# CHAINNEVERLIU/Pytorch-RL-EnhancedStableBaselines

Hardware: AMD Instinct MI355X
Metric: env-steps/sec (SAC, two-series CSTR, 4096 vec-envs) at 1/2/4/8 GPUs (higher is better)
Workload: dtype f32; 1 GPU; SAC MlpPolicy class defaults on 4096 vectorised two-series CSTR envs per GPU (obs 4/act 2, euler, batch 256, ring 244x4096, 1 gradient step per vec-step; hipGraph replay, 8 iterations per graph); n_envs_per_gpu=4096, global_batch=256, parallelism=dp1, hip_graph=True, hip_graph_requested=True, graph_unroll=8, blas=rocblas, n_updates=2370

## Files before the change

include/cstr_rl_hip.h:

```cpp
#ifndef CSTR_RL_HIP_H
#define CSTR_RL_HIP_H

#include <stdint.h>

#ifdef __cplusplus
extern "C" {
#endif

#define CSTR_ABI_VERSION 5

#define CSTR_OK 0
#define CSTR_E_BADARG (-1)
#define CSTR_E_UNSUPPORTED (-2)

#define CSTR_INTEGRATOR_EULER 0
#define CSTR_INTEGRATOR_RK4 1

typedef void *cstr_stream_t;

typedef struct cstr_coef {
    float q_v1, q_v2, cf, tf, tcf, k0, neg_e, r_gas, hk, rho_cp, cool1, cool2, neg_ua1, neg_ua2, rho_c, c_pc, dt;
    float s_lo[4], s_hi[4], s_span[4];
    float a_lo[2], a_hi[2], a_span[2];
    float target_c2, conc_span;
// ... 327 lines not shown
                         const cstr_sac_head_fin_t *fin, int tiles, cstr_stream_t stream);

typedef struct cstr_chain_root {
    int32_t mode, batch;
    float gamma, scale;
    const float *q_part[4];
    const float *b3[4];
    int32_t n_parts, reserved;
    const float *next_logp, *rew, *done;
    const float *ent_coef;
    const float *logp;
    float *target_out;
    float *q_out;
    float *gq_out;
    float *loss_out, *loss_sum;
    cstr_alpha_part_t alpha;
    uint64_t *rng_ctl;
    uint64_t rng_advance;
    int64_t *adam_advance[2];
    double adam_beta1[2], adam_beta2[2];
} cstr_chain_root_t;
int cstr_q_chain_bwd_f32(const cstr_chain_net_t *nets, int n_nets, const cstr_chain_root_t *root, int w_in, int obs_dim, int h1, int h2,
                         float *dz2, float *dz1, float *gact_part, int tiles, cstr_stream_t stream);

int cstr_chain_sum_parts_f32(const float *part, int n_parts, int64_t rows, int cols, float *out, int64_t out_stride, cstr_stream_t stream);

int cstr_sac_actor_chain_bwd_f32(const cstr_sac_actor_t *actor, const float *gact_part, int n_nets, int n_parts, const float *ent_coef,
                                 const float *x_pi, const float *params, const float *eps, const float *a_h1, const float *a_h2,
                                 float *g_params, float *dz2, float *dz1, int64_t batch, int kind, int tiles, cstr_stream_t stream);

#define CSTR_BCQ_MAX_LATENT 256
#define CSTR_BCQ_MAX_ACT 64
#define CSTR_BCQ_MAX_SAMPLES 4096
#define CSTR_BCQ_MAX_ROWS 16777216
int cstr_bcq_latent_fwd_f32(const float *params, int64_t ldp, const float *obs, int64_t ldo, const float *eps_in, uint64_t *rng_ctl,
                            float *xdec, int64_t ldx, float *std_out, float *eps_out, int64_t batch, int obs_dim, int latent,
                            cstr_stream_t stream);
int cstr_bcq_vae_loss_f32(const float *recon, int64_t ldr, const float *act, int64_t lda, const float *params, int64_t ldp,
                          const float *std, int64_t batch, int act_dim, int latent, float *g_recon, float *g_mean, float *g_std,
                          float *loss_out, float *loss_sum, cstr_stream_t stream);
int cstr_bcq_latent_bwd_f32(const float *g_z, int64_t ldg, const float *g_mean_kl, const float *g_std_kl, const float *params, int64_t ldp,
                            const float *std, const float *eps, float *g_params, int64_t batch, int latent, cstr_stream_t stream);
int cstr_bcq_expand_f32(const float *state, int64_t lds, int64_t n_states, int samples, int obs_dim, int latent, const float *noise,
                        uint64_t *rng_ctl, float clip, float *xdec, int64_t ldx, float *xa, int64_t lda, float *xb, int64_t ldb,
                        cstr_stream_t stream);
int cstr_bcq_perturb_fwd_f32(const float *a_vae, int64_t lda, const float *p, int64_t ldp, float max_perturbation, float *out, int64_t ldo,
// ... 141 lines not shown
```

pytorch-rl-enhancedstablebaselines_amd/core/_native.py:

```python
import ctypes as C
import os
from typing import Optional

_PKG_ROOT = os.path.dirname(os.path.dirname(os.path.abspath(__file__)))
LIB_PATH = os.environ.get("CSTR_LIB_PATH", os.path.join(_PKG_ROOT, "libcstr_rl_hip.so"))

INTEGRATORS = {"euler": 0, "rk4": 1}
RING_CTL_WORDS, ADAM_CTL_WORDS, MT_STATE_WORDS, PCG_STATE_WORDS, MAX_SAMPLE_BATCH = 4, 4, 628, 4, 16384
MAX_NOISE_PERIOD = 8
VECNORM_STATE_WORDS = 20
RNG_CTL_WORDS, MAX_HEAD_ACT, MAX_LINEAR_SETS, MAX_ADAM_SEGS = 16, 4, 16, 4
MAX_ENS_CRITICS = 16
SDE_MAX_LATENT, SDE_MAX_MATS = 4096, 65537
BCQ_MAX_LATENT, BCQ_MAX_ACT, BCQ_MAX_SAMPLES, BCQ_MAX_ROWS = 256, 64, 4096, 1 << 24
ROLLOUT_CTL_WORDS, PPO_WS_WORDS, PPO_MAX_BLOCKS, PPO_MAX_ROWS = 4, 1024, 64, 1 << 30
DQN_MAX_LEVELS = 16
HER_STRATEGIES = {"future": 0, "final": 1, "episode": 2}
HER_MAX_BATCH, HER_MAX_ROWS, HER_MAX_ENVS, HER_GOAL_TAG = 1024, 8192, 1 << 24, 0x90A17A67

SYMBOLS = (
    "cstr_abi_version", "cstr_error_string", "cstr_default_coef", "cstr_vec_step_f32", "cstr_reset_draw_f32",
    "cstr_replay_add_f32", "cstr_collect_step_f32", "cstr_collect_step_rng_f32", "cstr_mt19937_seed", "cstr_mt19937_normal_f32", "cstr_mt19937_normal_f64", "cstr_replay_sample_mt19937_f32", "cstr_replay_sample_packed_mt19937_f32", "cstr_replay_gather_packed_f32", "cstr_rollout_step_f32", "cstr_linear_act_fwd_gather_f32",
    "cstr_adam_multi_f32", "cstr_gaussian_head_fwd_f32", "cstr_gaussian_head_gemm_fwd_f32", "cstr_gaussian_head_bwd_f32", "cstr_gaussian_head_bwd_input_f32", "cstr_linear_act_fwd_f32", "cstr_linear_act_fwd_sets_f32", "cstr_linear_bwd_input_f32", "cstr_linear_bwd_weight_f32", "cstr_linear_bwd_weight_sets_f32", "cstr_td_twin_q_loss_f32", "cstr_policy_rows_fwd_f32", "cstr_policy_swizzle_f32", "cstr_target_smooth_f32", "cstr_linear_smooth_fwd_f32", "cstr_hidden_head_fwd_f32", "cstr_hidden_head_bwd_f32", "cstr_hidden_head_bwd_root_f32", "cstr_vecnorm_init_f64", "cstr_vecnorm_step_f64", "cstr_vecnorm_apply_f32",
    "cstr_td_target_min_f32", "cstr_polyak_f32", "cstr_adam_f32", "cstr_bias_act_fwd_f32", "cstr_bias_act_bwd_f32", "cstr_bias_act_bwd_rows_f32",
    "cstr_squashed_gaussian_fwd_f32", "cstr_squashed_gaussian_bwd_f32", "cstr_sac_alpha_f32", "cstr_twin_q_loss_f32",
    "cstr_sac_actor_loss_f32", "cstr_neg_mean_loss_f32", "cstr_td_ens_q_loss_f32", "cstr_sac_actor_ens_loss_f32",
    "cstr_sac_actor_chain_fwd_f32", "cstr_q_chain_fwd_f32", "cstr_q_chain_bwd_f32", "cstr_sac_actor_chain_bwd_f32",
    "cstr_linear_bwd_weight_adam_sets_f32", "cstr_wgrad_adam_lean", "cstr_wgrad_adam_tile_body", "cstr_chain_sum_parts_f32",
    "cstr_sde_draw_f32", "cstr_sde_head_fwd_f32", "cstr_sde_head_bwd_f32", "cstr_sde_param_grad_f32",
    "cstr_bcq_latent_fwd_f32", "cstr_bcq_vae_loss_f32", "cstr_bcq_latent_bwd_f32", "cstr_bcq_expand_f32", "cstr_bcq_perturb_fwd_f32",
    "cstr_bcq_perturb_bwd_f32", "cstr_bcq_target_f32", "cstr_bcq_select_f32",
    "cstr_diag_gaussian_act_f32", "cstr_rollout_add_f32", "cstr_gae_f32", "cstr_ppo_gather_f32", "cstr_ppo_loss_f32", "cstr_grad_clip_f32",
    "cstr_a2c_loss_f32", "cstr_rmsprop_f32",
    "cstr_mt19937_rand_flag_f64", "cstr_dqn_act_f32", "cstr_dqn_loss_f32",
    "cstr_eval_episodes_f32",
    "cstr_categorical_act_f32", "cstr_categorical_loss_f32",
    "cstr_goal_vec_step_f32", "cstr_her_add_f32", "cstr_her_sample_f32",
)


class Coef(C.Structure):
    _fields_ = [(n, C.c_float) for n in (
        "q_v1", "q_v2", "cf", "tf", "tcf", "k0", "neg_e", "r_gas", "hk", "rho_cp", "cool1", "cool2", "neg_ua1",
        "neg_ua2", "rho_c", "c_pc", "dt")] + [
        ("s_lo", C.c_float * 4), ("s_hi", C.c_float * 4), ("s_span", C.c_float * 4),
        ("a_lo", C.c_float * 2), ("a_hi", C.c_float * 2), ("a_span", C.c_float * 2),
        ("target_c2", C.c_float), ("conc_span", C.c_float), ("max_steps", C.c_int32)]


class Ring(C.Structure):
    _fields_ = [(n, C.c_void_p) for n in ("obs", "next_obs", "act", "rew", "done", "timeout")] + [
# ... 165 lines not shown
```

pytorch-rl-enhancedstablebaselines_amd/core/common/hip_ops.py:

```python
import ctypes as C
from typing import Optional

import torch as th

from core import _native as nv
from core._native import INTEGRATORS, check, ptr, stream_ptr


def _chk(t: th.Tensor, name: str, shape, dtype) -> th.Tensor:
    if not isinstance(t, th.Tensor):
        raise TypeError(f"{name}: expected a torch.Tensor, got {type(t)}")
    if not t.is_cuda:
        raise ValueError(f"{name}: must live in HBM (device tensor); got device {t.device}. No CPU fallback exists.")
    if t.device.index != th.cuda.current_device():
        raise ValueError(f"{name}: lives on {t.device}, the current device is cuda:{th.cuda.current_device()}")
    if t.dtype != dtype:
        raise ValueError(f"{name}: dtype {t.dtype}, expected {dtype}")
    if tuple(t.shape) != tuple(shape):
        raise ValueError(f"{name}: shape {tuple(t.shape)}, expected {tuple(shape)}")
    if not t.is_contiguous():
        raise ValueError(f"{name}: must be contiguous")
    return t


# ... 1231 lines not shown
               rng_advance=None, adam_advance=()) -> "nv.ChainRoot":
    part = nv.AlphaPart()
    if alpha is not None:
        part = nv.AlphaPart(alpha["log_alpha"].data_ptr(), alpha["logp_pi"].data_ptr(), float(alpha["target_entropy"]), alpha["grad_out"].data_ptr(),
                            alpha["ent_coef_out"].data_ptr(), *(_dp(alpha.get(k)) for k in ("loss_out", "loss_sum", "ent_coef_sum")))
    qp, bb = (C.c_void_p * 4)(), (C.c_void_p * 4)()
    for i, (q, b) in enumerate(zip(q_parts, b3s)):
        qp[i], bb[i] = q.data_ptr(), b.data_ptr()
    rc_ptr, adv = (None, 0) if rng_advance is None else (rng_advance[0].data_ptr(), int(rng_advance[1]))
    actl, ab1, ab2 = (C.c_void_p * 2)(), (C.c_double * 2)(), (C.c_double * 2)()
    for i, opt in enumerate(adam_advance):
        actl[i], (ab1[i], ab2[i]) = opt.ctl.data_ptr(), opt.param_groups[0]["betas"]
    return nv.ChainRoot({"td": 1, "sac_actor": 2, "neg_mean": 3}[mode], batch, float(gamma), float(scale), qp, bb, n_parts, 0, _dp(next_logp), _dp(rew),
                        _dp(done), None if alpha is not None else _dp(ent_coef), _dp(logp), _dp(target_out), _dp(q_out), _dp(gq_out), _dp(loss_out),
                        _dp(loss_sum), part, rc_ptr, adv, actl, ab1, ab2)


def q_chain_bwd(nets, root: "nv.ChainRoot", w_in: int, obs_dim: int, h1: int, h2: int, tiles: int, dz2=None, dz1=None, gact_part=None):
    arr = (nv.ChainNet * len(nets))(*nets)
    check(nv.lib().cstr_q_chain_bwd_f32(arr, C.c_int(len(nets)), C.byref(root), C.c_int(w_in), C.c_int(obs_dim), C.c_int(h1), C.c_int(h2), ptr(dz2),
                                        ptr(dz1), ptr(gact_part), C.c_int(tiles), stream_ptr()), "cstr_q_chain_bwd_f32")


def sac_actor_chain_bwd(actor: "nv.SacActorNet", gact_part, n_nets: int, n_parts: int, ent_coef, x_pi, params, eps, a_h1, a_h2, g_params, dz2, dz1,
                        batch: int, tiles: int, kind: int = 0):
    hn = actor.act_dim if kind == nv.CHAIN_HEAD_DETERMINISTIC else 2 * actor.act_dim
    _chk(gact_part, "gact_part", (n_nets, n_parts, batch, actor.act_dim), th.float32)
    _chk(g_params, "g_params", (batch, hn), th.float32), _chk(dz2, "dz2", (batch, actor.h2), th.float32)
    _chk(dz1, "dz1", (batch, actor.h1), th.float32)
    check(nv.lib().cstr_sac_actor_chain_bwd_f32(C.byref(actor), ptr(gact_part), C.c_int(n_nets), C.c_int(n_parts), ptr(ent_coef), ptr(x_pi), ptr(params),
                                                ptr(eps), ptr(a_h1), ptr(a_h2), ptr(g_params), ptr(dz2), ptr(dz1), C.c_int64(batch), C.c_int(kind),
                                                C.c_int(tiles), stream_ptr()), "cstr_sac_actor_chain_bwd_f32")


def chain_sum_parts(part, out):
    rows, cols = out.shape
    n_parts = part.numel() // (rows * cols)
    if part.numel() != n_parts * rows * cols or _f32c(part, "part") is None:
        raise ValueError("part: needs [n_parts, rows, cols]")
    if not (out.is_cuda and out.dtype == th.float32 and out.stride(1) == 1):
        raise ValueError("out: needs a float32 device matrix with unit inner stride")
    check(nv.lib().cstr_chain_sum_parts_f32(ptr(part), C.c_int(n_parts), C.c_int64(rows), C.c_int(cols), ptr(out), C.c_int64(out.stride(0)), stream_ptr()),
          "cstr_chain_sum_parts_f32")


PPO_SCALARS = ("policy_gradient_loss", "value_loss", "entropy_loss", "loss", "approx_kl", "clip_fraction")
# ... 313 lines not shown
```

pytorch-rl-enhancedstablebaselines_amd/csrc/cstr_chain.hip:

```cpp
#include <hip/hip_runtime.h>
#include <stdint.h>

#include "../../include/cstr_rl_hip.h"
#include "cstr_device.h"
#include "cstr_rng_device.h"

namespace {

using f32x4 = __attribute__((ext_vector_type(4))) float;
typedef unsigned int u32x4 __attribute__((ext_vector_type(4)));
constexpr int BUF_OOB = 0x40000000;
constexpr int CH_THREADS = 256, CH_WAVES = 4;
constexpr float LOG_STD_MIN = -20.0f, LOG_STD_MAX = 2.0f;
constexpr int MAX_A = CSTR_MAX_HEAD_ACT;

constexpr int SM_PART = 0;
constexpr int SM_RED = SM_PART + 3 * 64 * 4;
constexpr int SM_XS = SM_RED + 4 * 16 * 8;
constexpr int SM_GS = SM_XS + 16 * 16;
constexpr int SM_PANEL = SM_GS + 16 * 8;
static size_t chain_lds_bytes(int k, int w1_pad) { return (size_t)(SM_PANEL + 16 * (k + 4) + w1_pad * k) * sizeof(float); }

__device__ __forceinline__ __amdgpu_buffer_rsrc_t rsrc_of(const float *base, const int64_t floats)
{
// ... 778 lines not shown
#pragma unroll
        for (int e = 0; e < 4; ++e) a.dz1[((int64_t)g * B + m0 + 4 * h + e) * H1 + k0 + r] = d[e];
    }
    if (a.dz2) {
        const int cpg = (H2 + gridDim.x - 1) / gridDim.x;
#pragma unroll
        for (int i = 0; i < 2; ++i) {
            const int c = t + CH_THREADS * i;
            if (c < H2 && c / cpg == (int)blockIdx.x) {
#pragma unroll
                for (int row = 0; row < 16; ++row) a.dz2[((int64_t)g * B + m0 + row) * H2 + c] = y[i][row];
            }
        }
    }
    if (t < 16 && blockIdx.x == 0) {
        const int row = m0 + t;
        if (rt.q_out) rt.q_out[(int64_t)g * B + row] = o_q;
        if (rt.gq_out) rt.gq_out[(int64_t)g * B + row] = o_gq;
        if (rt.mode == 1 && g == 0 && rt.target_out) rt.target_out[row] = o_tq;
    }
    CH_STAMP(2, 7);
}

struct ActorBwdArgs {
    cstr_sac_actor_t net;
    const float *gact_part; int n_nets, n_parts; const float *ent_coef;
    const float *x_pi, *params, *eps, *a_h1, *a_h2;
    float *g_params, *dz2, *dz1;
    int batch, tiles, kind;
};

template <int D, int A, int NQ, int WX>
__global__ __launch_bounds__(CH_THREADS) void sac_actor_chain_bwd_kernel(const ActorBwdArgs a)
{
    extern __shared__ __align__(16) float smem[];
    constexpr int W = D + A;
    const int t = threadIdx.x, lane = t & 63, wave = t >> 6, r = lane & 15, h = lane >> 4;
    const int T = WX ? exact_tiles<NQ, WX>() : a.tiles, S = CH_WAVES / T, tile = wave % T, ks = wave / T;
    const int H1 = WX ? exact_h1<WX>() : a.net.h1, H2 = WX ? exact_h2<WX>() : a.net.h2, B = a.batch;
    const int k0 = (blockIdx.x * T + tile) * 16, m0 = blockIdx.y * 16;
    const bool col_ok = k0 + r < H1, det = a.kind == CSTR_CHAIN_HEAD_DETERMINISTIC;
    const int col = min(k0 + r, H1 - 1), HN = det ? A : 2 * A;
    float *gs = smem + SM_GS, *panel = smem + SM_PANEL;
    const int ld = H2 + 4;
    CH_STAMP(3, 0);
    float4 bq[NQ];
// ... 121 lines not shown
#define NQ_TOP_sac_actor_chain_bwd_kernel 16
#define CHAIN_DISPATCH(KERNEL, LAY, WXV, NQV, GRID, LDS, STREAM, ARGS)                             \
    do {                                                                                           \
        if ((LAY) == 0 && (WXV) == 1) CHAIN_NQ(KERNEL, 4, 2, 1, NQV, GRID, LDS, STREAM, ARGS);     \
        else if ((LAY) == 0 && (WXV) == 2) CHAIN_NQ(KERNEL, 4, 2, 2, NQV, GRID, LDS, STREAM, ARGS); \
        else if ((LAY) == 0) CHAIN_NQ(KERNEL, 4, 2, 0, NQV, GRID, LDS, STREAM, ARGS);              \
        else if ((LAY) == 1 && (WXV) == 1) CHAIN_NQ(KERNEL, 8, 2, 1, NQV, GRID, LDS, STREAM, ARGS); \
        else if ((LAY) == 1) CHAIN_NQ(KERNEL, 8, 2, 0, NQV, GRID, LDS, STREAM, ARGS);              \
        else if ((WXV) == 2) CHAIN_NQ(KERNEL, 8, 4, 2, NQV, GRID, LDS, STREAM, ARGS);              \
        else CHAIN_NQ(KERNEL, 8, 4, 0, NQV, GRID, LDS, STREAM, ARGS);                              \
    } while (0)

static int chain_wx(int h1, int h2, int tiles, int nq)
{
    static const bool off = getenv("CSTR_EXACT_SHAPES") && atoi(getenv("CSTR_EXACT_SHAPES")) == 0;
    if (off || (nq != 4 && nq != 8 && nq != 16)) return 0;
    if (h1 == 256 && h2 == 256 && nq == 4 * tiles) return 1;
    if (h1 == 400 && h2 == 300 && nq == 8 * tiles) return 2;
    return 0;
}

constexpr size_t CHAIN_LDS_LIMIT = 64 * 1024;

}

#ifdef CSTR_CHAIN_STAMPS
extern "C" int cstr_diag_chain_stamps(unsigned long long *host_out, int64_t words)
{
    return (int)hipMemcpyFromSymbol(host_out, HIP_SYMBOL(chain_stamps), (size_t)words * 8);
}
#endif

static int check_actor(const cstr_sac_actor_t *n)
{
    if (!n || !n->w1 || !n->b1 || !n->w2 || !n->b2 || !n->hw || !n->hb) return CSTR_E_BADARG;
    if (!((n->obs_dim == 4 && n->act_dim == 2) || (n->obs_dim == 8 && (n->act_dim == 2 || n->act_dim == 4)))) return CSTR_E_UNSUPPORTED;
    if (!aligned16(n->w1) || !aligned16(n->w2)) return CSTR_E_BADARG;
    return CSTR_OK;
}

extern "C" int cstr_sac_actor_chain_fwd_f32(const cstr_sac_actor_t *actor, const cstr_ring_t *ring, int64_t *ring_ctl, int advance_ring,
                                            const int32_t *sample_idx, int64_t batch, float *x_data, float *x_pi, float *x_next,
                                            float *out_done, float *out_rew, float *a_h1, float *a_h2, float *head_part,
                                            const uint64_t *head_rng_ctl, uint64_t head_rng_offset, float *eps_all, int rows_mode,
                                            int head_n, int tiles, cstr_stream_t stream)
{
// ... 42 lines not shown
        a.nets[g] = n;
    }
    if (fin) {
        if (!fin->head_part || !fin->hb || fin->n_parts < 1 || fin->act_dim < 1 || fin->act_dim > MAX_A || fin->obs_dim != obs_dim || fin->obs_dim + fin->act_dim != w_in)
            return CSTR_E_BADARG;
        const bool det = fin->kind == CSTR_CHAIN_HEAD_DETERMINISTIC;
        if (fin->kind != CSTR_CHAIN_HEAD_GAUSSIAN && !det) return CSTR_E_BADARG;
        if (fin->part_rows < batch || fin->next_offset < 0 || fin->next_offset + batch > fin->part_rows) return CSTR_E_BADARG;
        if (!det && (!fin->eps || !fin->x_pi || !fin->x_next || !fin->params || !fin->logp_pi || !fin->logp_next)) return CSTR_E_BADARG;
        for (int g = 0; g < n_nets; ++g) {
            const int role = nets[g].role;
            if ((role == CSTR_CHAIN_ROLE_NEXT_STORE && !fin->x_next) || ((role == CSTR_CHAIN_ROLE_STORE_PI || role == CSTR_CHAIN_ROLE_PI) && !fin->x_pi))
                return CSTR_E_BADARG;
        }
        a.fin = *fin;
        a.has_fin = 1;
    }
    a.n_nets = n_nets; a.h1 = h1; a.h2 = h2; a.batch = (int)batch; a.tiles = tiles;
    const dim3 grid((unsigned)((h2 + 16 * tiles - 1) / (16 * tiles)), (unsigned)(batch / 16), (unsigned)n_nets);
    const size_t lds = chain_lds_bytes(h1, (w_in % 2 == 0 && w_in + 1 <= 16) ? 0 : (w_in + 1 <= 8 ? 8 : 16));
    const int nq = nq_for(h1, tiles, 32), lay = chain_layout(obs_dim, w_in - obs_dim);
    if (!nq || lay < 0 || lds > CHAIN_LDS_LIMIT) return CSTR_E_UNSUPPORTED;
    hipStream_t s = (hipStream_t)stream;
    CHAIN_DISPATCH(q_chain_fwd_kernel, lay, chain_wx(h1, h2, tiles, nq), nq, grid, lds, s, a);
    return (int)hipGetLastError();
}

extern "C" int cstr_q_chain_bwd_f32(const cstr_chain_net_t *nets, int n_nets, const cstr_chain_root_t *root, int w_in, int obs_dim, int h1,
                                    int h2, float *dz2, float *dz1, float *gact_part, int tiles, cstr_stream_t stream)
{
    if (!nets || !root || n_nets < 1 || n_nets > 2 || w_in < 1 || w_in > 12 || obs_dim < 0 || obs_dim > w_in) return CSTR_E_BADARG;
    if (root->mode < 1 || root->mode > 3 || root->n_parts < 1) return CSTR_E_BADARG;
    if ((root->mode == 3) != (n_nets == 1)) return CSTR_E_BADARG;
    if (!chain_dims_ok(h1, h2, root->batch, tiles)) return CSTR_E_UNSUPPORTED;
        QBwdArgs a = {};
    for (int g = 0; g < n_nets; ++g) {
        const cstr_chain_net_t &n = nets[g];
        if (!n.w1 || !n.w2 || !n.w3 || !n.h1 || !n.h2) return CSTR_E_BADARG;
        a.nets[g] = n;
    }
    const int need = root->mode == 1 ? 4 : n_nets;
    for (int g = 0; g < need; ++g)
        if (!root->q_part[g] || !root->b3[g]) return CSTR_E_BADARG;
    if (root->mode == 1 && (!root->rew || !root->done)) return CSTR_E_BADARG;
    if (root->mode == 2 && (!root->logp || !root->ent_coef)) return CSTR_E_BADARG;
    if (root->mode == 1 && root->alpha.log_alpha && (!root->alpha.logp_pi || !root->alpha.grad_out || !root->alpha.ent_coef_out)) return CSTR_E_BADARG;
    a.root = *root;
    a.n_nets = n_nets; a.h1 = h1; a.h2 = h2; a.tiles = tiles;
    a.dz2 = dz2; a.dz1 = dz1; a.gact_part = gact_part;
    const dim3 grid((unsigned)((h1 + 16 * tiles - 1) / (16 * tiles)), (unsigned)(root->batch / 16 + 1), (unsigned)n_nets);
    const size_t lds = chain_lds_bytes(h2, 0);
    const int nq = nq_for(h2, tiles), lay = chain_layout(obs_dim, w_in - obs_dim);
    if (!nq || lay < 0 || lds > CHAIN_LDS_LIMIT) return CSTR_E_UNSUPPORTED;
    hipStream_t s = (hipStream_t)stream;
    CHAIN_DISPATCH(q_chain_bwd_kernel, lay, chain_wx(h1, h2, tiles, nq), nq, grid, lds, s, a);
    return (int)hipGetLastError();
}

extern "C" int cstr_chain_sum_parts_f32(const float *part, int n_parts, int64_t rows, int cols, float *out, int64_t out_stride, cstr_stream_t stream)
{
    if (!part || !out || n_parts < 1 || rows < 1 || cols < 1 || out_stride < cols) return CSTR_E_BADARG;
    if ((int64_t)n_parts * rows * cols >= (1 << 28)) return CSTR_E_UNSUPPORTED;
    const int64_t n = rows * cols;
    chain_sum_parts_kernel<<<(unsigned)((n + 255) / 256), 256, 0, (hipStream_t)stream>>>(part, n_parts, rows, cols, out, out_stride);
    return (int)hipGetLastError();
}

extern "C" int cstr_sac_actor_chain_bwd_f32(const cstr_sac_actor_t *actor, const float *gact_part, int n_nets, int n_parts,
                                            const float *ent_coef, const float *x_pi, const float *params, const float *eps, const float *a_h1,
                                            const float *a_h2, float *g_params, float *dz2, float *dz1, int64_t batch, int kind, int tiles,
                                            cstr_stream_t stream)
{
    const int rc = check_actor(actor);
    if (rc) return rc;
    if (kind != CSTR_CHAIN_HEAD_GAUSSIAN && kind != CSTR_CHAIN_HEAD_DETERMINISTIC) return CSTR_E_BADARG;
    if (!gact_part || n_nets < 1 || n_nets > 2 || n_parts < 1 || !x_pi || !a_h1 || !a_h2 || !g_params || !dz2 || !dz1) return CSTR_E_BADARG;
    if (kind == CSTR_CHAIN_HEAD_GAUSSIAN && (!ent_coef || !params || !eps)) return CSTR_E_BADARG;
    if (!chain_dims_ok(actor->h1, actor->h2, batch, tiles)) return CSTR_E_UNSUPPORTED;
    ActorBwdArgs a = {};
// ... 13 lines not shown
```

Before: 71.74 million env-steps/s.

## Add lean specialized Q-chain forward/backward kernels with compile-time mode dispatch

Adds templated lean variants of the Q-network chain forward and backward kernels. They are specialized at compile time on head kind, loss mode, alpha and next-logp presence, and part-count buckets. Partial sums are fetched through buffer loads issued early, and uniform pointers are pinned into scalar registers, aiming to cut argument-struct loads, branching and latency inside the hot SAC critic/actor chain kernels. A runtime toggle, on by default, falls back to the original kernels for unsupported shapes. The cost is many more template instantiations and the risk that the hand-duplicated code diverges from the original semantics.

New measurement: 73.23 million env-steps/s (median of 6 runs). 1.02x the previous value.

```diff
diff --git a/include/cstr_rl_hip.h b/include/cstr_rl_hip.h
--- a/include/cstr_rl_hip.h
+++ b/include/cstr_rl_hip.h
@@ -373,6 +373,7 @@
 } cstr_chain_root_t;
 int cstr_q_chain_bwd_f32(const cstr_chain_net_t *nets, int n_nets, const cstr_chain_root_t *root, int w_in, int obs_dim, int h1, int h2,
                          float *dz2, float *dz1, float *gact_part, int tiles, cstr_stream_t stream);
+int cstr_chain_lean(int on);
 
 int cstr_chain_sum_parts_f32(const float *part, int n_parts, int64_t rows, int cols, float *out, int64_t out_stride, cstr_stream_t stream);
 
diff --git a/pytorch-rl-enhancedstablebaselines_amd/core/_native.py b/pytorch-rl-enhancedstablebaselines_amd/core/_native.py
--- a/pytorch-rl-enhancedstablebaselines_amd/core/_native.py
+++ b/pytorch-rl-enhancedstablebaselines_amd/core/_native.py
@@ -26,7 +26,7 @@
     "cstr_squashed_gaussian_fwd_f32", "cstr_squashed_gaussian_bwd_f32", "cstr_sac_alpha_f32", "cstr_twin_q_loss_f32",
     "cstr_sac_actor_loss_f32", "cstr_neg_mean_loss_f32", "cstr_td_ens_q_loss_f32", "cstr_sac_actor_ens_loss_f32",
     "cstr_sac_actor_chain_fwd_f32", "cstr_q_chain_fwd_f32", "cstr_q_chain_bwd_f32", "cstr_sac_actor_chain_bwd_f32",
-    "cstr_linear_bwd_weight_adam_sets_f32", "cstr_wgrad_adam_lean", "cstr_wgrad_adam_tile_body", "cstr_chain_sum_parts_f32",
+    "cstr_linear_bwd_weight_adam_sets_f32", "cstr_wgrad_adam_lean", "cstr_wgrad_adam_tile_body", "cstr_chain_lean", "cstr_chain_sum_parts_f32",
     "cstr_sde_draw_f32", "cstr_sde_head_fwd_f32", "cstr_sde_head_bwd_f32", "cstr_sde_param_grad_f32",
     "cstr_bcq_latent_fwd_f32", "cstr_bcq_vae_loss_f32", "cstr_bcq_latent_bwd_f32", "cstr_bcq_expand_f32", "cstr_bcq_perturb_fwd_f32",
     "cstr_bcq_perturb_bwd_f32", "cstr_bcq_target_f32", "cstr_bcq_select_f32",
diff --git a/pytorch-rl-enhancedstablebaselines_amd/core/common/hip_ops.py b/pytorch-rl-enhancedstablebaselines_amd/core/common/hip_ops.py
--- a/pytorch-rl-enhancedstablebaselines_amd/core/common/hip_ops.py
+++ b/pytorch-rl-enhancedstablebaselines_amd/core/common/hip_ops.py
@@ -1277,6 +1277,10 @@
                                         ptr(dz1), ptr(gact_part), C.c_int(tiles), stream_ptr()), "cstr_q_chain_bwd_f32")
 
 
+def chain_lean(on: int = -1) -> int:
+    return int(nv.lib().cstr_chain_lean(C.c_int(on)))
+
+
 def sac_actor_chain_bwd(actor: "nv.SacActorNet", gact_part, n_nets: int, n_parts: int, ent_coef, x_pi, params, eps, a_h1, a_h2, g_params, dz2, dz1,
                         batch: int, tiles: int, kind: int = 0):
     hn = actor.act_dim if kind == nv.CHAIN_HEAD_DETERMINISTIC else 2 * actor.act_dim
diff --git a/pytorch-rl-enhancedstablebaselines_amd/csrc/cstr_chain.hip b/pytorch-rl-enhancedstablebaselines_amd/csrc/cstr_chain.hip
--- a/pytorch-rl-enhancedstablebaselines_amd/csrc/cstr_chain.hip
+++ b/pytorch-rl-enhancedstablebaselines_amd/csrc/cstr_chain.hip
@@ -824,6 +824,401 @@
     CH_STAMP(2, 7);
 }
 
+template <int NP>
+struct PartBatchN {
+    float v[NP];
+    __device__ __forceinline__ void request(const float *part, const int n, const int64_t stride, const int64_t at, const int64_t total, const bool on = true)
+    {
+        const __amdgpu_buffer_rsrc_t rs = rsrc_of(part, total);
+        const unsigned st = (unsigned)stride, at0 = (unsigned)at;
+#pragma unroll
+        for (int p = 0; p < NP; ++p) v[p] = ld32(rs, (on && p < n) ? (int)(4u * (p * st + at0)) : BUF_OOB);
+    }
+    __device__ __forceinline__ float sum() const
+    {
+        float s = v[0];
+#pragma unroll
+        for (int p = 1; p < NP; ++p) s += v[p];
+        return s;
+    }
+};
+__device__ __forceinline__ float ld_uniform(const float *p) { return ld32(rsrc_of(p, 1), 0); }
+
+constexpr int part_bucket_row(const int n) { return n <= 8 ? 8 : 16; }
+constexpr int part_bucket_loss(const int n) { return n <= 4 ? 4 : n <= 8 ? 8 : 16; }
+
+enum { QF_PLAIN = 0, QF_GAUSSIAN = 1, QF_DETERMINISTIC = 2 };
+struct QFwdLeanArgs {
+    cstr_chain_net_t nets[CSTR_CHAIN_MAX_NETS];
+    float *x_pi, *x_next, *params, *logp_pi, *logp_next;
+};
+
+template <int D, int A, int NQ, int FIN, int PB>
+__global__ __launch_bounds__(CH_THREADS) void q_chain_fwd_lean_kernel(const int batch, const int fin_parts, const float *fin_head_part, const float *fin_hb,
+                                                                      const float *fin_eps, const int fin_part_rows, const int fin_next_offset,
+                                                                      const float fin_sigma, const float fin_clip, const unsigned long long roles,
+                                                                      const QFwdLeanArgs a)
+{
+    extern __shared__ __align__(16) float smem[];
+    constexpr int W = D + A, WX = 1;
+    const int t = threadIdx.x, lane = t & 63, wave = t >> 6, r = lane & 15, h = lane >> 4;
+    constexpr int T = exact_tiles<NQ, WX>(), S = CH_WAVES / T;
+    const int tile = wave % T, ks = wave / T;
+    const cstr_chain_net_t net = a.nets[blockIdx.z];
+    float *const o_x_pi = a.x_pi, *const o_x_next = a.x_next, *const o_params = a.params, *const o_logp_pi = a.logp_pi, *const o_logp_next = a.logp_next;
+    __builtin_amdgcn_sched_barrier(0);
+    constexpr int H1 = exact_h1<WX>(), H2 = exact_h2<WX>();
+    const int B = batch;
+    const int n0 = (blockIdx.x * T + tile) * 16, m0 = blockIdx.y * 16;
+    float *xs = smem + SM_XS, *red = smem + SM_RED, *panel = smem + SM_PANEL;
+    constexpr int ld = H1 + 4;
+    float *w1s = panel + 16 * ld;
+    const bool col_ok = n0 + r < H2;
+    CH_STAMP(1, 0);
+    const int role = FIN != QF_PLAIN ? (int)((roles >> (4 * blockIdx.z)) & 15u) : CSTR_CHAIN_ROLE_PLAIN;
+    const bool nxt = role == CSTR_CHAIN_ROLE_NEXT || role == CSTR_CHAIN_ROLE_NEXT_STORE;
+    const bool own = nxt || role == CSTR_CHAIN_ROLE_PI;
+    const bool fin_rows = own || (role == CSTR_CHAIN_ROLE_STORE_PI && blockIdx.x == 0);
+    const bool fin_lane = FIN != QF_PLAIN && fin_rows && t < 16 * A;
+    const int f_row = t / A, f_j = t % A;
+    constexpr bool f_det = FIN == QF_DETERMINISTIC;
+    PartBatchN<PB> p_mu, p_raw;
+    float f_ev = 0.0f, f_hb_mu = 0.0f, f_hb_raw = 0.0f;
+    constexpr int HN = f_det ? A : 2 * A;
+    const int64_t f_i = (nxt ? fin_next_offset : 0) + m0 + f_row;
+    if (FIN != QF_PLAIN) {
+        const int64_t pstride = (int64_t)fin_part_rows * HN, ptotal = pstride * fin_parts;
+        p_mu.request(fin_head_part, fin_parts, pstride, f_i * HN + f_j, ptotal, fin_lane);
+        if (!f_det) p_raw.request(fin_head_part, fin_parts, pstride, f_i * HN + A + f_j, ptotal, fin_lane);
+    }
+    asm volatile("" ::"s"(net.w1), "s"(net.b1), "s"(net.w2), "s"(net.b2), "s"(net.w3), "s"(net.x), "s"(net.h1), "s"(net.h2), "s"(net.q_part));
+    if (FIN != QF_PLAIN) asm volatile("" ::"s"(o_x_pi), "s"(o_x_next), "s"(o_params), "s"(o_logp_pi), "s"(o_logp_next));
+    if (fin_lane) {
+        f_ev = (!f_det || fin_eps) ? fin_eps[f_i * A + f_j] : 0.0f;
+        f_hb_mu = fin_hb[f_j];
+        f_hb_raw = f_det ? 0.0f : fin_hb[A + f_j];
+    }
+    float4 bq[NQ];
+    load_b_fwd<NQ>(bq, net.w2, H2, H1, n0, ks, S);
+    const int col = min(n0 + r, H2 - 1);
+    const float bv = net.b2[col];
+    const float w3v = col_ok ? net.w3[col] : 0.0f;
+    stage_w1<W>(w1s, net.w1, net.b1, H1);
+    L1Direct<W> l1d;
+    if (l1_pad<W>() == 0) l1d.request(net.w1, net.b1, H1);
+    {
+        const int row = t >> 4, k = t & 15;
+        float xv = k == W ? 1.0f : 0.0f;
+        if (k < W && !(own && k >= D)) xv = net.x[(int64_t)(m0 + row) * W + k];
+        if (!(own && k >= D && k < W)) xs[row * 16 + k] = xv;
+    }
+    float f_mu = 0.0f, f_raw = 0.0f, f_a = 0.0f, f_lp = 0.0f;
+    if (fin_lane) {
+        const float ev = f_ev;
+        f_mu = p_mu.sum() + f_hb_mu;
+        if (f_det) {
+            f_a = tanhf(f_mu);
+            if (nxt) f_a = fminf(fmaxf(f_a + fminf(fmaxf(ev * fin_sigma, -fin_clip), fin_clip), -1.0f), 1.0f);
+        } else {
+            f_raw = p_raw.sum() + f_hb_raw;
+            float term;
+            sample_action(f_mu, f_raw, ev, f_a, term);
+            f_lp = term;
+            if (A >= 2) f_lp += __shfl_xor(f_lp, 1, 64);
+            if (A == 4) f_lp += __shfl_xor(f_lp, 2, 64);
+        }
+        if (own) xs[f_row * 16 + D + f_j] = f_a;
+    }
+    CH_STAMP(1, 1);
+    lds_barrier();
+    CH_STAMP(1, 2);
+    layer1_mfma<l1_pad<W>(), W>(xs, w1s, panel, ld, H1, &l1d, net.w1, net.b1);
+    lds_barrier();
+    CH_STAMP(1, 3);
+    f32x4 acc = tile_mma<NQ>(panel, ld, H1, bq, ks, S);
+    CH_STAMP(1, 4);
+    acc = combine_split_k(acc, smem, T, S);
+    CH_STAMP(1, 5);
+    float hv[4] = {0.0f, 0.0f, 0.0f, 0.0f};
+    if (wave < T) {
+#pragma unroll
+        for (int e = 0; e < 4; ++e) {
+            hv[e] = col_ok ? fmaxf(acc[e] + bv, 0.0f) : 0.0f;
+#ifdef CSTR_HEAD_F64
+            double sd = (double)hv[e] * (double)w3v;
+            sd += __shfl_xor(sd, 8, 64); sd += __shfl_xor(sd, 4, 64); sd += __shfl_xor(sd, 2, 64); sd += __shfl_xor(sd, 1, 64);
+            const float s = (float)sd;
+#else
+            const float s = rowsum16(hv[e] * w3v);
+#endif
+            if (r == 0) red[(tile * 16 + 4 * h + e) * 8] = s;
+        }
+    }
+    lds_barrier();
+    CH_STAMP(1, 6);
+    if (t < 16) {
+        float s = red[t * 8];
+#pragma unroll
+        for (int tl = 1; tl < T; ++tl) s += red[(tl * 16 + t) * 8];
+        net.q_part[(int64_t)blockIdx.x * B + m0 + t] = s;
+    }
+    if (wave < T && col_ok && net.h2) {
+#pragma unroll
+        for (int e = 0; e < 4; ++e) net.h2[(int64_t)(m0 + 4 * h + e) * H2 + n0 + r] = hv[e];
+    }
+    if (blockIdx.x == 0 && net.h1) store_panel(panel, ld, net.h1, H1, m0);
+    if (fin_lane && blockIdx.x == 0 && role != CSTR_CHAIN_ROLE_NEXT) {
+        const int bb = m0 + f_row;
+        (nxt ? o_x_next : o_x_pi)[(int64_t)bb * W + D + f_j] = f_a;
+        if (!nxt && !f_det) {
+            o_params[(int64_t)bb * 2 * A + f_j] = f_mu;
+            o_params[(int64_t)bb * 2 * A + A + f_j] = f_raw;
+        }
+        if (f_j == 0 && !f_det) (nxt ? o_logp_next : o_logp_pi)[bb] = f_lp;
+    }
+    CH_STAMP(1, 7);
+}
+
+template <int LB>
+__device__ __forceinline__ float q_from_parts_n(const float *part, const float *b3, const int n_parts, const int batch, const int row)
+{
+    const float b = b3[0];
+    return sum_parts_n<LB>(rsrc_of(part, (int64_t)n_parts * batch), n_parts, batch, row) + b;
+}
+
+template <int MODE, bool ALPHA, bool NLOGP, int LB>
+__device__ __forceinline__ void chain_loss_lean(const cstr_chain_root_t &rt, float *sm)
+{
+    const int tid = threadIdx.x, B = rt.batch, P = rt.n_parts;
+    constexpr bool with_alpha = MODE == 1 && ALPHA;
+    const float la = with_alpha ? rt.alpha.log_alpha[0] : 0.0f;
+    const float ec = with_alpha ? expf(la) : (rt.ent_coef ? rt.ent_coef[0] : 0.0f);
+    const float inv = 1.0f / (float)B;
+    if (MODE == 1) {
+        float a1 = 0.0f, a2 = 0.0f, aa = 0.0f;
+        for (int b = tid; b < B; b += 256) {
+            float q = fminf(q_from_parts_n<LB>(rt.q_part[2], rt.b3[2], P, B, b), q_from_parts_n<LB>(rt.q_part[3], rt.b3[3], P, B, b));
+            if (NLOGP) q = q - ec * rt.next_logp[b];
+            const float tq = rt.rew[b] + (1.0f - rt.done[b]) * rt.gamma * q;
+            const float d1 = q_from_parts_n<LB>(rt.q_part[0], rt.b3[0], P, B, b) - tq, d2 = q_from_parts_n<LB>(rt.q_part[1], rt.b3[1], P, B, b) - tq;
+            a1 += d1 * d1;
+            a2 += d2 * d2;
+            if (with_alpha) aa += rt.alpha.logp_pi[b] + rt.alpha.target_entropy;
+        }
+        const float s1 = block_sum_256(a1, sm), s2 = block_sum_256(a2, sm);
+        const float mean = with_alpha ? block_sum_256(aa, sm) / (float)B : 0.0f;
+        if (tid == 0) {
+            const float loss = rt.scale * (s1 / (float)B + s2 / (float)B);
+            if (rt.loss_out) rt.loss_out[0] = loss;
+            if (rt.loss_sum) rt.loss_sum[0] += loss;
+            if (with_alpha) {
+                rt.alpha.grad_out[0] = -mean;
+                rt.alpha.ent_coef_out[0] = ec;
+                if (rt.alpha.loss_out) rt.alpha.loss_out[0] = -(la * mean);
+                if (rt.alpha.loss_sum) rt.alpha.loss_sum[0] += -(la * mean);
+                if (rt.alpha.ent_coef_sum) rt.alpha.ent_coef_sum[0] += ec;
+            }
+        }
+    } else if (MODE == 3) {
+        float acc = 0.0f;
+        for (int b = tid; b < B; b += 256) acc += q_from_parts_n<LB>(rt.q_part[0], rt.b3[0], P, B, b);
+        const float sum = block_sum_256(acc, sm);
+        if (tid == 0) {
+            const float loss = -(sum * inv);
+            if (rt.loss_out) rt.loss_out[0] = loss;
+            if (rt.loss_sum) rt.loss_sum[0] += loss;
+        }
+    } else {
+        float acc = 0.0f;
+        for (int b = tid; b < B; b += 256) {
+            const float x = q_from_parts_n<LB>(rt.q_part[0], rt.b3[0], P, B, b), c = q_from_parts_n<LB>(rt.q_part[1], rt.b3[1], P, B, b);
+            acc += ec * rt.logp[b] - (x <= c ? x : c);
+        }
+        const float sum = block_sum_256(acc, sm);
+        if (tid == 0) {
+            const float loss = sum * inv;
+            if (rt.loss_out) rt.loss_out[0] = loss;
+            if (rt.loss_sum) rt.loss_sum[0] += loss;
+        }
+    }
+    if (tid == 0 && rt.rng_ctl) rt.rng_ctl[1] += rt.rng_advance;
+    if (tid < 2 && rt.adam_advance[tid]) {
+        int64_t *ctl = rt.adam_advance[tid];
+        double *pw = reinterpret_cast<double *>(ctl + 2);
+        ctl[0] += 1;
+        pw[0] *= rt.adam_beta1[tid];
+        pw[1] *= rt.adam_beta2[tid];
+    }
+}
+
+struct QBwdLeanNet { const float *w1, *w2, *w3, *h1, *h2; };
+struct QBwdLeanArgs {
+    QBwdLeanNet nets[2];
+    const float *b3[4];
+    const float *ec_src;
+    const float *rew, *done, *next_logp;
+    float *dz2, *dz1, *gact_part, *q_out, *gq_out, *target_out;
+    float gamma, scale;
+    cstr_chain_root_t root;
+};
+
+template <int D, int A, int NQ, int MODE, bool ALPHA, bool NLOGP, int LB>
+__global__ __launch_bounds__(CH_THREADS) void q_chain_bwd_lean_kernel(const int batch, const int n_parts, const float *qp0, const float *qp1, const float *qp2,
+                                                                      const float *qp3, const QBwdLeanArgs a)
+{
+    extern __shared__ __align__(16) float smem[];
+    constexpr int W = D + A, WX = 1;
+    constexpr bool GACT = MODE != 1;
+    constexpr int NEED = MODE == 1 ? 4 : MODE == 3 ? 1 : 2;
+    constexpr int PB = part_bucket_row(LB);
+    const int t = threadIdx.x, lane = t & 63, wave = t >> 6, r = lane & 15, h = lane >> 4;
+    const int B = batch;
+    constexpr int H1 = exact_h1<WX>(), H2 = exact_h2<WX>();
+    const int g = blockIdx.z;
+    if (__builtin_expect((int)blockIdx.y == B / 16, 0)) {
+        if (g == 0 && blockIdx.x == 0) chain_loss_lean<MODE, ALPHA, NLOGP, LB>(a.root, smem + SM_RED);
+        return;
+    }
+    constexpr int T = exact_tiles<NQ, WX>(), S = CH_WAVES / T;
+    const int tile = wave % T, ks = wave / T;
+    const QBwdLeanNet net = a.nets[g];
+    const float *const b3p[4] = {a.b3[0], a.b3[1], a.b3[2], a.b3[3]};
+    const float *const ec_src = a.ec_src, *const rew = a.rew, *const done = a.done, *const next_logp = a.next_logp;
+    float *const o_dz2 = a.dz2, *const o_dz1 = a.dz1, *const o_gact = a.gact_part, *const o_q = a.q_out, *const o_gqp = a.gq_out, *const o_tqp = a.target_out;
+    const float gamma = a.gamma, scale = a.scale;
+    const int k0 = (blockIdx.x * T + tile) * 16, m0 = blockIdx.y * 16;
+    const bool col_ok = k0 + r < H1;
+    const int col = min(k0 + r, H1 - 1);
+    float *red = smem + SM_RED, *gs = smem + SM_GS, *panel = smem + SM_PANEL;
+    constexpr int ld = H2 + 4;
+    CH_STAMP(2, 0);
+    const float *const qp[4] = {qp0, qp1, qp2, qp3};
+    PartBatchN<PB> pq[NEED];
+    if (t < 16) {
+#pragma unroll
+        for (int q = 0; q < NEED; ++q) pq[q].request(qp[q], n_parts, B, m0 + t, (int64_t)n_parts * B);
+    }
+    asm volatile("" ::"s"(net.w1), "s"(net.w2), "s"(net.w3), "s"(net.h1), "s"(net.h2), "s"(b3p[0]), "s"(o_q), "s"(o_gqp), "s"(scale));
+    if (NEED > 1) asm volatile("" ::"s"(b3p[1]));
+    if (MODE == 1) asm volatile("" ::"s"(b3p[2]), "s"(b3p[3]), "s"(o_dz2), "s"(o_dz1), "s"(o_tqp), "s"(gamma), "s"(rew), "s"(done));
+    if (MODE == 1 && NLOGP) asm volatile("" ::"s"(ec_src), "s"(next_logp));
+    if (GACT) asm volatile("" ::"s"(o_gact));
+    float r_nl = 0.0f, r_rw = 0.0f, r_dn = 0.0f, r_b3[4] = {0.0f, 0.0f, 0.0f, 0.0f}, r_ec = 0.0f;
+    if (t < 16) {
+        const int row = m0 + t;
+#pragma unroll
+        for (int q = 0; q < NEED; ++q) r_b3[q] = ld_uniform(b3p[q]);
+        if (MODE == 1) {
+            if (NLOGP) {
+                r_nl = next_logp[row];
+                r_ec = ld_uniform(ec_src);
+            }
+            r_rw = rew[row];
+            r_dn = done[row];
+        }
+    }
+    float4 bq[NQ];
+    load_b_bwd<NQ>(bq, net.w2, H2, H1, k0, ks, S);
+    float ty[4];
+#pragma unroll
+    for (int e = 0; e < 4; ++e) ty[e] = net.h1[(int64_t)(m0 + 4 * h + e) * H1 + col];
+    float w1a[A];
+#pragma unroll
+    for (int j = 0; j < A; ++j) w1a[j] = GACT ? net.w1[(int64_t)col * W + D + j] : 0.0f;
+    float y[16];
+    const float w3c = net.w3[t];
+#pragma unroll
+    for (int row = 0; row < 16; ++row) y[row] = net.h2[(int64_t)(m0 + row) * H2 + t];
+    float o_qv = 0.0f, o_gq = 0.0f, o_tq = 0.0f;
+    if (t < 16) {
+        const float kq = scale * 2.0f / (float)B, inv = 1.0f / (float)B;
+        if constexpr (MODE == 1) {
+            const float ec = ALPHA ? expf(r_ec) : r_ec;
+            const float qa = pq[2].sum() + r_b3[2], qb = pq[3].sum() + r_b3[3];
+            o_qv = (g == 0 ? pq[0].sum() + r_b3[0] : pq[1].sum() + r_b3[1]);
+            float q = fminf(qa, qb);
+            if (NLOGP) q = q - ec * r_nl;
+            o_tq = r_rw + (1.0f - r_dn) * gamma * q;
+            o_gq = kq * (o_qv - o_tq);
+        } else if constexpr (MODE == 3) {
+            o_qv = pq[0].sum() + r_b3[0];
+            o_gq = -inv;
+        } else {
+            const float q1 = pq[0].sum() + r_b3[0], q2 = pq[1].sum() + r_b3[1];
+            const bool first = q1 <= q2;
+            o_qv = g == 0 ? q1 : q2;
+            o_gq = (first == (g == 0)) ? -inv : 0.0f;
+        }
+        gs[t] = o_gq;
+    }
+    CH_STAMP(2, 1);
+    lds_barrier();
+    CH_STAMP(2, 2);
+    {
+        float gq[16];
+#pragma unroll
+        for (int q = 0; q < 4; ++q) {
+            const float4 g4 = *reinterpret_cast<const float4 *>(gs + 4 * q);
+            gq[4 * q] = g4.x; gq[4 * q + 1] = g4.y; gq[4 * q + 2] = g4.z; gq[4 * q + 3] = g4.w;
+        }
+#pragma unroll
+        for (int row = 0; row < 16; ++row) {
+            y[row] = y[row] > 0.0f ? gq[row] * w3c : 0.0f;
+            panel[row * ld + t] = y[row];
+        }
+    }
+    lds_barrier();
+    CH_STAMP(2, 3);
+    f32x4 acc = tile_mma<NQ>(panel, ld, H2, bq, ks, S);
+    CH_STAMP(2, 4);
+    acc = combine_split_k(acc, smem, T, S);
+    CH_STAMP(2, 5);
+    float d[4] = {0.0f, 0.0f, 0.0f, 0.0f};
+    if (wave < T) {
+#pragma unroll
+        for (int e = 0; e < 4; ++e) d[e] = (col_ok && ty[e] > 0.0f) ? acc[e] : 0.0f;
+        if (GACT) {
+#pragma unroll
+            for (int j = 0; j < A; ++j) {
+#pragma unroll
+                for (int e = 0; e < 4; ++e) {
+                    const float s = rowsum16(d[e] * w1a[j]);
+                    if (r == 0) red[(tile * 16 + 4 * h + e) * 8 + j] = s;
+                }
+            }
+        }
+    }
+    if (GACT) {
+        lds_barrier();
+        if (t < 16 * A) {
+            const int row = t / A, j = t % A;
+            float s = red[row * 8 + j];
+#pragma unroll
+            for (int tl = 1; tl < T; ++tl) s += red[(tl * 16 + row) * 8 + j];
+            o_gact[(((int64_t)g * gridDim.x + blockIdx.x) * B + m0 + row) * A + j] = s;
+        }
+    }
+    CH_STAMP(2, 6);
+    if (!GACT) {
+        if (wave < T && col_ok) {
+#pragma unroll
+            for (int e = 0; e < 4; ++e) o_dz1[((int64_t)g * B + m0 + 4 * h + e) * H1 + k0 + r] = d[e];
+        }
+        const int cpg = (H2 + gridDim.x - 1) / gridDim.x;
+        if (t / cpg == (int)blockIdx.x) {
+#pragma unroll
+            for (int row = 0; row < 16; ++row) o_dz2[((int64_t)g * B + m0 + row) * H2 + t] = y[row];
+        }
+    }
+    if (t < 16 && blockIdx.x == 0) {
+        const int row = m0 + t;
+        if (o_q) o_q[(int64_t)g * B + row] = o_qv;
+        if (o_gqp) o_gqp[(int64_t)g * B + row] = o_gq;
+        if (MODE == 1 && g == 0 && o_tqp) o_tqp[row] = o_tq;
+    }
+    CH_STAMP(2, 7);
+}
+
 struct ActorBwdArgs {
     cstr_sac_actor_t net;
     const float *gact_part; int n_nets, n_parts; const float *ent_coef;
@@ -991,6 +1386,120 @@
 
 constexpr size_t CHAIN_LDS_LIMIT = 64 * 1024;
 
+int chain_lean_enabled = 1;
+
+struct QFwdLeanScalars { int batch, parts; const float *head_part, *hb, *eps; int part_rows, next_offset; float sigma, clip; unsigned long long roles; };
+
+template <int D, int A, int NQ, int FIN, int PB>
+void q_fwd_lean_go(const dim3 grid, const size_t lds, hipStream_t s, const QFwdLeanScalars &c, const QFwdLeanArgs &a)
+{
+    q_chain_fwd_lean_kernel<D, A, NQ, FIN, PB><<<grid, CH_THREADS, lds, s>>>(c.batch, c.parts, c.head_part, c.hb, c.eps, c.part_rows, c.next_offset, c.sigma,
+                                                                             c.clip, c.roles, a);
+}
+template <int D, int A, int NQ>
+void q_fwd_lean_variant(const int finv, const int pb, const dim3 grid, const size_t lds, hipStream_t s, const QFwdLeanScalars &c, const QFwdLeanArgs &a)
+{
+    if (finv == QF_PLAIN) q_fwd_lean_go<D, A, NQ, QF_PLAIN, 8>(grid, lds, s, c, a);
+    else if (finv == QF_GAUSSIAN && pb == 8) q_fwd_lean_go<D, A, NQ, QF_GAUSSIAN, 8>(grid, lds, s, c, a);
+    else if (finv == QF_GAUSSIAN) q_fwd_lean_go<D, A, NQ, QF_GAUSSIAN, 16>(grid, lds, s, c, a);
+    else if (pb == 8) q_fwd_lean_go<D, A, NQ, QF_DETERMINISTIC, 8>(grid, lds, s, c, a);
+    else q_fwd_lean_go<D, A, NQ, QF_DETERMINISTIC, 16>(grid, lds, s, c, a);
+}
+template <int D, int A, typename... Rest>
+void q_fwd_lean_nq(const int nq, Rest &&...rest)
+{
+    if (nq == 4) q_fwd_lean_variant<D, A, 4>(rest...);
+    else if (nq == 8) q_fwd_lean_variant<D, A, 8>(rest...);
+    else q_fwd_lean_variant<D, A, 16>(rest...);
+}
+
+enum { QB_TD_ALPHA = 0, QB_TD_LOGP = 1, QB_TD_PLAIN = 2, QB_ACTOR_SAC = 3, QB_ACTOR_NEG_MEAN = 4 };
+struct QBwdLeanScalars { int batch, parts; const float *qp[4]; };
+
+template <int D, int A, int NQ, int MODE, bool ALPHA, bool NLOGP, int LB>
+void q_bwd_lean_go(const dim3 grid, const size_t lds, hipStream_t s, const QBwdLeanScalars &c, const QBwdLeanArgs &a)
+{
+    q_chain_bwd_lean_kernel<D, A, NQ, MODE, ALPHA, NLOGP, LB><<<grid, CH_THREADS, lds, s>>>(c.batch, c.parts, c.qp[0], c.qp[1], c.qp[2], c.qp[3], a);
+}
+template <int D, int A, int NQ, int LB>
+void q_bwd_lean_variant(const int variant, const dim3 grid, const size_t lds, hipStream_t s, const QBwdLeanScalars &c, const QBwdLeanArgs &a)
+{
+    if (variant == QB_TD_ALPHA) q_bwd_lean_go<D, A, NQ, 1, true, true, LB>(grid, lds, s, c, a);
+    else if (variant == QB_TD_LOGP) q_bwd_lean_go<D, A, NQ, 1, false, true, LB>(grid, lds, s, c, a);
+    else if (variant == QB_TD_PLAIN) q_bwd_lean_go<D, A, NQ, 1, false, false, LB>(grid, lds, s, c, a);
+    else if (variant == QB_ACTOR_SAC) q_bwd_lean_go<D, A, NQ, 2, false, false, LB>(grid, lds, s, c, a);
+    else q_bwd_lean_go<D, A, NQ, 3, false, false, LB>(grid, lds, s, c, a);
+}
+template <int D, int A, int NQ, typename... Rest>
+void q_bwd_lean_lb(const int lb, Rest &&...rest)
+{
+    if (lb == 4) q_bwd_lean_variant<D, A, NQ, 4>(rest...);
+    else if (lb == 8) q_bwd_lean_variant<D, A, NQ, 8>(rest...);
+    else q_bwd_lean_variant<D, A, NQ, 16>(rest...);
+}
+template <int D, int A, typename... Rest>
+void q_bwd_lean_nq(const int nq, Rest &&...rest)
+{
+    if (nq == 4) q_bwd_lean_lb<D, A, 4>(rest...);
+    else if (nq == 8) q_bwd_lean_lb<D, A, 8>(rest...);
+    else q_bwd_lean_lb<D, A, 16>(rest...);
+}
+
+bool q_fwd_lean_launch(const QFwdArgs &g, const int lay, const int wx, const int nq, const dim3 grid, const size_t lds, hipStream_t s)
+{
+    if (!chain_lean_enabled || wx != 1 || (lay != 0 && lay != 1)) return false;
+    if (g.has_fin && g.fin.n_parts > MAX_PARTS) return false;
+    QFwdLeanArgs a = {};
+    QFwdLeanScalars c = {};
+    c.batch = g.batch;
+    for (int i = 0; i < g.n_nets; ++i) {
+        a.nets[i] = g.nets[i];
+        c.roles |= (unsigned long long)(g.nets[i].role & 15) << (4 * i);
+    }
+    int finv = QF_PLAIN, pb = 8;
+    if (g.has_fin) {
+        const cstr_sac_head_fin_t &f = g.fin;
+        finv = f.kind == CSTR_CHAIN_HEAD_DETERMINISTIC ? QF_DETERMINISTIC : QF_GAUSSIAN;
+        pb = part_bucket_row(f.n_parts);
+        c.parts = f.n_parts; c.head_part = f.head_part; c.hb = f.hb; c.eps = f.eps; c.part_rows = f.part_rows; c.next_offset = f.next_offset;
+        c.sigma = f.sigma; c.clip = f.clip;
+        a.x_pi = f.x_pi; a.x_next = f.x_next; a.params = f.params; a.logp_pi = f.logp_pi; a.logp_next = f.logp_next;
+    }
+    if (lay == 0) q_fwd_lean_nq<4, 2>(nq, finv, pb, grid, lds, s, c, a);
+    else q_fwd_lean_nq<8, 2>(nq, finv, pb, grid, lds, s, c, a);
+    return true;
+}
+
+bool q_bwd_lean_launch(const QBwdArgs &g, const int lay, const int wx, const int nq, const dim3 grid, const size_t lds, hipStream_t s)
+{
+    const cstr_chain_root_t &rt = g.root;
+    if (!chain_lean_enabled || wx != 1 || (lay != 0 && lay != 1) || rt.n_parts > MAX_PARTS) return false;
+    const bool stores_dz = g.dz1 && g.dz2 && !g.gact_part, stores_gact = g.gact_part && !g.dz1 && !g.dz2;
+    const bool alpha = rt.alpha.log_alpha != nullptr, nlogp = rt.next_logp != nullptr;
+    int variant;
+    if (rt.mode == 1) {
+        if (!stores_dz || (alpha && !nlogp) || (!alpha && nlogp && !rt.ent_coef)) return false;
+        variant = alpha ? QB_TD_ALPHA : nlogp ? QB_TD_LOGP : QB_TD_PLAIN;
+    } else {
+        if (!stores_gact) return false;
+        variant = rt.mode == 2 ? QB_ACTOR_SAC : QB_ACTOR_NEG_MEAN;
+    }
+    QBwdLeanArgs a = {};
+    QBwdLeanScalars c = {};
+    for (int i = 0; i < g.n_nets; ++i) a.nets[i] = QBwdLeanNet{g.nets[i].w1, g.nets[i].w2, g.nets[i].w3, g.nets[i].h1, g.nets[i].h2};
+    for (int q = 0; q < 4; ++q) { a.b3[q] = rt.b3[q]; c.qp[q] = rt.q_part[q]; }
+    a.ec_src = alpha ? rt.alpha.log_alpha : rt.ent_coef;
+    a.dz2 = g.dz2; a.dz1 = g.dz1; a.gact_part = g.gact_part; a.q_out = rt.q_out; a.gq_out = rt.gq_out; a.target_out = rt.target_out;
+    a.gamma = rt.gamma; a.scale = rt.scale;
+    a.root = rt;
+    a.rew = rt.rew; a.done = rt.done; a.next_logp = rt.next_logp;
+    c.batch = rt.batch; c.parts = rt.n_parts;
+    const int lb = part_bucket_loss(rt.n_parts);
+    if (lay == 0) q_bwd_lean_nq<4, 2>(nq, lb, variant, grid, lds, s, c, a);
+    else q_bwd_lean_nq<8, 2>(nq, lb, variant, grid, lds, s, c, a);
+    return true;
+}
+
 }
 
 #ifdef CSTR_CHAIN_STAMPS
@@ -1079,7 +1588,8 @@
     const int nq = nq_for(h1, tiles, 32), lay = chain_layout(obs_dim, w_in - obs_dim);
     if (!nq || lay < 0 || lds > CHAIN_LDS_LIMIT) return CSTR_E_UNSUPPORTED;
     hipStream_t s = (hipStream_t)stream;
-    CHAIN_DISPATCH(q_chain_fwd_kernel, lay, chain_wx(h1, h2, tiles, nq), nq, grid, lds, s, a);
+    const int wx = chain_wx(h1, h2, tiles, nq);
+    if (!q_fwd_lean_launch(a, lay, wx, nq, grid, lds, s)) CHAIN_DISPATCH(q_chain_fwd_kernel, lay, wx, nq, grid, lds, s, a);
     return (int)hipGetLastError();
 }
 
@@ -1110,8 +1620,16 @@
     const int nq = nq_for(h2, tiles), lay = chain_layout(obs_dim, w_in - obs_dim);
     if (!nq || lay < 0 || lds > CHAIN_LDS_LIMIT) return CSTR_E_UNSUPPORTED;
     hipStream_t s = (hipStream_t)stream;
-    CHAIN_DISPATCH(q_chain_bwd_kernel, lay, chain_wx(h1, h2, tiles, nq), nq, grid, lds, s, a);
+    const int wx = chain_wx(h1, h2, tiles, nq);
+    if (!q_bwd_lean_launch(a, lay, wx, nq, grid, lds, s)) CHAIN_DISPATCH(q_chain_bwd_kernel, lay, wx, nq, grid, lds, s, a);
     return (int)hipGetLastError();
+}
+
+extern "C" int cstr_chain_lean(int on)
+{
+    const int was = chain_lean_enabled;
+    if (on >= 0) chain_lean_enabled = on != 0;
+    return was;
 }
 
 extern "C" int cstr_chain_sum_parts_f32(const float *part, int n_parts, int64_t rows, int cols, float *out, int64_t out_stride, cstr_stream_t stream)
```
